# fkluger/vanishing_points_2017

Hardware: AMD Instinct MI355X
Metric: images/sec (LSD->CNN->EM) + horizon-AUC parity, YUD-shape, 1/2/4/8 GPU (higher is better)
Workload: dtype f32 (CNN: f32 operands / accumulation / results; conv1 multiply EXACT bf16 pieces of the f32 operands (three per operand) on the bf16 matrix cores; conv2-5, fc6 and fc7 multiply scaled fp16 PAIRS of the f32 operands (22 of 24 significand bits, three exact products per f32 product) on the fp16 matrix

## Files before the change

vanishing_points_2017_amd/csrc/em_device.hpp:

```cpp
#ifndef VPK_EM_DEVICE_HPP_
#define VPK_EM_DEVICE_HPP_

#include "wave_prims.hpp"
#include "../../include/vpk.h"
#include "em_layout.hpp"

namespace vpk {

constexpr int MAXM = 64;
constexpr int GRIDN = 20;
constexpr int NCELL = GRIDN * GRIDN;
constexpr int MAXCOMP = 100;
constexpr int MT = 8;
constexpr int PART_DOUBLES = 2048;
constexpr int WT_DOUBLES = 6144;
constexpr int KNN1 = 10;
constexpr int TRACE_COLS = 12;
constexpr int KNN2 = 4;
constexpr double PI_D = 3.141592653589793238462643383279502884;

struct Shared {
    double cur[MAXM * 3];
    double nxt[MAXM * 3];
    double s[MAXM];
    double pv[MAXM];
    double vx[MAXM], vy[MAXM];
    double k2[MAXM];
    double cnt[MAXM], cntw[MAXM], err[MAXM];
    int removed[MAXM];
    int icnt[MAXM];
    double red_v[32];
    int red_i[32];
    double pma[MAXCOMP], pmb[MAXCOMP], pw[MAXCOMP];
    float wts[NCELL];
    unsigned char mx[NCELL];
    int ncomp;
    int M;
    int status;
    unsigned flags;
    int ibuf[8];
    double dbuf[16];
    double sigma_prior;
    double active_us;
};

constexpr size_t SH_BYTES = (sizeof(Shared) + 15) / 16 * 16;
static_assert(sizeof(Shared) % 8 == 0 && sizeof(Shared) <= EM_STATE_DOUBLES * 8, "Shared must fit the slot's state region");
VPK_DEV Shared& SH() { return *reinterpret_cast<Shared*>(lds_base()); }
VPK_DEV double* WT() { return reinterpret_cast<double*>(lds_base() + SH_BYTES); }
VPK_DEV double* SCRATCH() { return WT(); }

struct EmCtx {
    int N;
    int ldn;
    int ld;
    int mcap;
    gdp l;
    cgdp lp;
    cgfp cnn;
    cgbp sphere;
    int ssize;
    cgdp init_vp;
    int n_init;
    vpk_em_params prm;
    gdp lsim;
    gdp pdist;
    gdp den;
    gdp lweight;
    gdp langle;
    gdp lscore;
    gdp lvsq;
    gdp pvl;
    gdp w;
    gdp wsrc;
    gdp drow;
    gdp cl;
    gip assoc;
    gip idx;
    gdp rowsum;
    int wt_doubles;
    gdp part;
    gdp lcopy;
    gdp lpcopy;
// ... 1233 lines not shown
        constexpr int RB = 4;
        const int nbatch = (M + RB - 1) / RB;
        for (int item = tid(); item < N * nbatch; item += nthreads()) {
            const int t0 = (item / N) * RB, kk = item - (item / N) * N;
            const double blw = bias * c.lweight[kk], dn = c.den[kk];
            cgdp pcol = c.part + kk;
            double v[RB][8];
#pragma unroll
            for (int u = 0; u < RB; ++u)
#pragma unroll
                for (int r = 0; r < 8; ++r)
                    v[u][r] = (t0 + u < M && r < R) ? pcol[((size_t)r * c.mcap + t0 + u) * c.ldn] : 0.0;
#pragma unroll
            for (int u = 0; u < RB; ++u) {
                if (t0 + u >= M) break;
                double sum = 0.0;
#pragma unroll
                for (int r = 0; r < 8; ++r) sum += v[u][r];
                c.w[(size_t)(m0 + t0 + u) * c.ldn + kk] = (wt[(size_t)kk * W + t0 + u] + blw * sum) / dn;
            }
        }
    }
    block_sync();
    if (tid() == 0) sh.dbuf[10] += lap(tq_);
}

VPK_DEVFN void zero_tail_rows(EmCtx& c) {
    const int N = c.N, jend = 8 * rs_jchunk(N);
    for (int p = tid(); p < (jend - N) * c.ld; p += nthreads()) c.lsim[(size_t)N * c.ld + p] = 0.0;
    block_sync();
}

template <int NT>
VPK_DEVFN void smooth_rows(EmCtx& c, int m0) {
    Shared& sh = SH();
    constexpr int W = NT * MT;
    constexpr int UNR = 4;
    const int N = uniform_int(c.N);
    m0 = uniform_int(m0);
    const int M = uniform_int(sh.M) - m0 < W ? uniform_int(sh.M) - m0 : W;
    const double bias = c.prm.wbias;
    double* wt = WT();
    long long tq_ = clock_ticks();
    const int jch = rs_jchunk(N), S = rs_sstride(jch, W);
    if (m0 != 0 || sh.ibuf[5] != RS_PANEL_FLAG + W) {
        for (int p = tid(); p < N * W; p += nthreads()) {
            const int j = p / W, m = p - j * W;
            wt[rs_row(j, jch, S, W) + m] = (m < M) ? c.wsrc[(size_t)j * c.mcap + m0 + m] : 0.0;
        }
        for (int p = N * W + tid(); p < 8 * jch * W; p += nthreads()) {
            const int j = p / W;
            wt[rs_row(j, jch, S, W) + (p - j * W)] = 0.0;
        }
        block_sync();
    }
    if (tid() == 0) sh.dbuf[8] += lap(tq_);
    double* red = wt + rs_panel_doubles(jch, W) + wave_id() * RS_RED_DOUBLES;
    const int d = lane() >> 4, i = lane() & 15;
    const int jA0 = d * jch, jB0 = (d + 4) * jch;
    const double* oA = wt + (size_t)d * S + i;
    const double* oB = wt + (size_t)(d + 4) * S + i;
    const size_t ld = (size_t)uniform_int(c.ld), ldn = (size_t)uniform_int(c.ldn);
    cgdp lsim = c.lsim, lweight = c.lweight, den = c.den;
    gdp wout = c.w;
    const int nb = (jch + UNR - 1) / UNR;
    cgdp lbase = uniform_ptr(lsim);
    const unsigned rowbytes = (unsigned)ld * 8u;
    const int kstep = uniform_int(nwaves()) * 16;
    int k0 = uniform_int(wave_id()) * 16;
    if (k0 < N) {
        int k = k0 + i;
        int kc = k < N ? k : N - 1;
        unsigned offA = ((unsigned)jA0 * (unsigned)ld + (unsigned)kc) * 8u, offB = ((unsigned)jB0 * (unsigned)ld + (unsigned)kc) * 8u;
        double aA[UNR], aB[UNR], nA_[UNR], nB_[UNR];
#pragma unroll
        for (int u = 0; u < UNR; ++u) {
            const int rn = u < jch ? u : jch - 1;
            cgdp rowp = (cgdp)((const VPK_GLOBAL char*)lbase + (size_t)rn * rowbytes);
            aA[u] = load_at(rowp, offA);
            aB[u] = load_at(rowp, offB);
        }
        for (;;) {
            const double lwk = lweight[kc];
            double dn = den[kc];
            const int k0n = k0 + kstep;
            const bool has_next = k0n < N;
            const int kn = k0n + i;
            const int kcn = has_next ? (kn < N ? kn : N - 1) : kc;
            const unsigned offAn = ((unsigned)jA0 * (unsigned)ld + (unsigned)kcn) * 8u, offBn = ((unsigned)jB0 * (unsigned)ld + (unsigned)kcn) * 8u;
            double accA[W], accB[W];
#pragma unroll
            for (int t = 0; t < W; ++t) { accA[t] = 0.0; accB[t] = 0.0; }
            double cA0 = oA[0], cA1 = W >= 24 ? oA[16] : 0.0, cB0 = oB[0], cB1 = W >= 24 ? oB[16] : 0.0;
            auto batch = [&](int b, double (&cuA)[UNR], double (&cuB)[UNR], double (&nxA)[UNR], double (&nxB)[UNR])
                             __attribute__((always_inline)) {
                const int r = b * UNR;
                const bool lastb = b + 1 == nb;
                const int nrow = lastb ? jch - r : UNR;
                const int rnext = lastb ? 0 : r + UNR;
                const unsigned oa = lastb ? offAn : offA, ob = lastb ? offBn : offB;
#pragma unroll
                for (int u = 0; u < UNR; ++u) {
                    int rn = rnext + u;
                    rn = rn < jch ? rn : jch - 1;
                    cgdp rowp = (cgdp)((const VPK_GLOBAL char*)lbase + (size_t)rn * rowbytes);
                    nxA[u] = load_at(rowp, oa);
                    nxB[u] = load_at(rowp, ob);
                }
#pragma unroll
                for (int u = 0; u < UNR; ++u) {
                    if (u < nrow) {
                        int rq = r + u + 1;
                        rq = rq < jch ? rq : 0;
                        const double* qA = oA + (size_t)rq * W;
                        const double* qB = oB + (size_t)rq * W;
                        const double xA0 = qA[0], xA1 = W >= 24 ? qA[16] : 0.0, xB0 = qB[0], xB1 = W >= 24 ? qB[16] : 0.0;
                        fmac8_row_bcast<0>(accA, cA0, cuA[u]);
                        if (W >= 16) fmac8_row_bcast<8>(accA + (W >= 16 ? 8 : 0), cA0, cuA[u]);
                        if (W >= 24) fmac8_row_bcast<0>(accA + (W >= 24 ? 16 : 0), cA1, cuA[u]);
// ... 196 lines not shown
            for (;;) {
                if (!step(va, vb)) break;
                if (!step(vb, va)) break;
            }
        }
    }
    if (tid() == 0) sh.dbuf[9] += lap(tq_);
#pragma unroll
    for (int cc = 0; cc < C; ++cc) {
        const int k = cc * WAVE + ln;
        if (k < N) {
#pragma unroll
            for (int q = 0; q < VPW; ++q) {
                const int t = wv + 8 * q;
                if (t < M) wout[(size_t)(m0 + t) * ldn + k] = (wreg[q][cc] + blwk[cc] * (tot[q][cc] + part[q][cc])) / dnk[cc];
            }
        }
    }
    block_sync();
    if (tid() == 0) sh.dbuf[10] += lap(tq_);
}
VPK_DEVFN void smooth_sparse_any(EmCtx& c, int m0) {
    switch (sp_cgroups(c.N)) {
        case 1: smooth_sparse<1>(c, m0); break;
        case 2: smooth_sparse<2>(c, m0); break;
        case 3: smooth_sparse<3>(c, m0); break;
        case 4: smooth_sparse<4>(c, m0); break;
        case 5: smooth_sparse<5>(c, m0); break;
        case 6: smooth_sparse<6>(c, m0); break;
        default: smooth_sparse<7>(c, m0); break;
    }
}

VPK_DEV void smooth_dispatch(EmCtx& c);
VPK_DEV void smooth(EmCtx& c) {
    smooth_dispatch(c);
    if (tid() == 0) SH().ibuf[5] = 0;
    block_sync();
}
VPK_DEV void smooth_dispatch(EmCtx& c) {
    Shared& sh = SH();
    const int M = sh.M, N = c.N;
    if (!c.prm.use_weights) {
        for (int m = 0; m < M; ++m)
            for (int k = tid(); k < N; k += nthreads()) c.w[(size_t)m * c.ldn + k] = c.wsrc[(size_t)k * c.mcap + m];
        block_sync();
        return;
    }
    if (M == 0) return;
    const int plan = smooth_plan(c, M);
    if (WAVE == 64 && (sh.ibuf[5] >= RS_PANEL_FLAG || plan == 2 || plan == 3)) {
        if (sparse_smoother_fits(c) && sh.ibuf[2] == 0) {
            for (int m0 = 0; m0 < M; m0 += 32) smooth_sparse_any(c, m0);
            return;
        }
        const int wpass = plan == 3 ? rs_wfit(c) : 32;
        for (int m0 = 0; m0 < M; m0 += wpass) {
            const int mm = (M - m0) < wpass ? (M - m0) : wpass;
            if (mm <= 8) smooth_rows<1>(c, m0);
            else if (mm <= 16) smooth_rows<2>(c, m0);
            else if (mm <= 24) smooth_rows<3>(c, m0);
            else smooth_rows<4>(c, m0);
        }
        return;
    }
    int wfit = (int)((c.wt_doubles / N) / MT) * MT;
    if (wfit > 32) wfit = 32;
    if (wfit >= MT) {
        for (int m0 = 0; m0 < M; m0 += wfit) {
            const int mm = (M - m0) < wfit ? (M - m0) : wfit;
            if (N > WAVE) {
                if (mm <= 8) smooth_full<1, 2>(c, m0);
                else if (mm <= 16) smooth_full<2, 2>(c, m0);
                else if (mm <= 24) smooth_full<3, 2>(c, m0);
                else smooth_full<4, 2>(c, m0);
            } else {
                if (mm <= 8) smooth_full<1, 1>(c, m0);
                else if (mm <= 16) smooth_full<2, 1>(c, m0);
                else if (mm <= 24) smooth_full<3, 1>(c, m0);
                else smooth_full<4, 1>(c, m0);
            }
        }
        return;
    }
    if (N > WAVE) smooth_blocks<2, 8>(c);
    else smooth_blocks<1, 4>(c);
}

VPK_DEVFN void assign_lines(EmCtx& c, bool hard) {
    Shared& sh = SH();
    const int M = sh.M, N = c.N;
    for (int n = tid(); n < N; n += nthreads()) {
        int best = 0;
        double bv = c.w[n];
        for (int m = 1; m < M; ++m) {
            double v = c.w[(size_t)m * c.ldn + n];
// ... 545 lines not shown
            } else {
                sh.flags |= VPK_EM_FLAG_VP_OVERFLOW;
            }
        }
    }
    if (tid() == 0) sh.dbuf[13] += lap(tq_);
    block_sync();
}

struct EmOut {
    double* vp;
    double* sigma;
    double* counts;
    double* counts_w;
    int* num_vp;
    long long* assoc;
    int* iterations;
    int* status;
    unsigned* flags;
    double* metric;
    double* trace;
    int max_vp;
    double* dbg = nullptr;
    double* d_pv = nullptr;
    double* d_angles = nullptr;
    double* d_pl = nullptr;
    double* d_plv = nullptr;
    double* d_pvl = nullptr;
    double* d_lvsq = nullptr;
};

VPK_DEVFN void write_result(EmCtx& c, EmOut& o, int status, int iterations) {
    Shared& sh = SH();
    const int N = c.N;
    int M = status == VPK_EM_OK ? sh.M : 0;
    if (M > o.max_vp) {
        M = o.max_vp;
        if (tid() == 0) sh.flags |= VPK_EM_FLAG_VP_OVERFLOW;
    }
    for (int m = tid(); m < o.max_vp; m += nthreads()) {
        bool ok = m < M;
        for (int d = 0; d < 3; ++d) o.vp[3 * m + d] = ok ? sh.nxt[3 * m + d] : 0.0;
        o.sigma[m] = ok ? sh.s[m] : 0.0;
        o.counts[m] = ok ? sh.cnt[m] : 0.0;
        o.counts_w[m] = ok ? sh.cntw[m] : 0.0;
    }
    for (int n = tid(); n < N; n += nthreads()) {
        int a = status == VPK_EM_OK ? c.assoc[n] : -1;
        o.assoc[n] = (a >= M) ? -1 : a;
        if (o.metric)
            for (int m = 0; m < o.max_vp; ++m)
                o.metric[(size_t)n * o.max_vp + m] = m < M ? c.w[(size_t)m * c.ldn + n] : 0.0;
    }
    if (o.d_pv) {
        for (int m = tid(); m < o.max_vp; m += nthreads()) {
            const bool ok = m < M;
            double alpha = 0.0, beta = 0.0;
            if (ok) {
                const double x0 = sh.nxt[3 * m], x1 = sh.nxt[3 * m + 1];
                beta = asin(x1);
                double inner = x0 / cos(beta);
                inner = inner < 1 ? inner : (is_nan(inner) ? inner : 1.0);
                inner = inner > -1 ? inner : (is_nan(inner) ? inner : -1.0);
                alpha = asin(inner);
            }
            o.d_pv[m] = ok ? sh.pv[m] : 0.0;
// ... 13 lines not shown
            }
            o.d_pl[n] = (pl > 1e-12 || is_nan(pl)) ? pl : 1e-12;
        }
    }
    block_sync();
    if (tid() == 0) {
        *o.num_vp = M;
        *o.iterations = iterations;
        *o.status = status;
        *o.flags = sh.flags;
    }
    block_sync();
}

VPK_DEV void trace_put(EmOut& o, int i, int slot, double v) {
    if (o.trace && tid() == 0) o.trace[TRACE_COLS * i + slot] = v;
}
VPK_DEV void trace_add(EmOut& o, int i, int slot, double v) {
    if (o.trace && tid() == 0) o.trace[TRACE_COLS * i + slot] += v;
}


constexpr int EM_DONE = 0, EM_SUSPENDED = 1;
constexpr long long EM_NO_DEADLINE = 0x7fffffffffffffffll;
struct EmSlice {
    long long deadline;
    int start_iter;
};

VPK_DEVFN void save_state(EmCtx& c) {
    typedef VPK_GLOBAL unsigned long long* gup;
    gup dst = (gup)c.state;
    const unsigned long long* src = reinterpret_cast<const unsigned long long*>(&SH());
    for (int q = tid(); q < (int)(sizeof(Shared) / 8); q += nthreads()) dst[q] = src[q];
    block_sync();
}
VPK_DEVFN void restore_state(EmCtx& c) {
    typedef const VPK_GLOBAL unsigned long long* cgup;
    cgup src = (cgup)c.state;
    unsigned long long* dst = reinterpret_cast<unsigned long long*>(&SH());
    block_sync();
    for (int q = tid(); q < (int)(sizeof(Shared) / 8); q += nthreads()) dst[q] = src[q];
    block_sync();
}

VPK_DEVFN int em_run(EmCtx& c, EmOut& o, EmSlice& sl) {
    Shared& sh = SH();
    const vpk_em_params& P = c.prm;
    const double max_stdd = 1e-6;
    const double merge_thresh_final = P.merge_thresh * 10;
    const int split_merge_it = 100;
    long long tk = clock_ticks();
    const long long t_begin = tk;
    int first = 0;
    if (sl.start_iter >= 0) {
        restore_state(c);
        first = sl.start_iter;
    } else {
    if (tid() == 0) { sh.flags = 0; sh.M = 0; sh.ncomp = 0; sh.ibuf[5] = 0; sh.ibuf[2] = 0; sh.active_us = 0; for (int q = 8; q < 16; ++q) sh.dbuf[q] = 0; }
    block_sync();
    if (o.trace)
        for (int q = tid(); q < TRACE_COLS * (P.num_iter + 1); q += nthreads()) o.trace[q] = 0.0;
    if (c.N <= 0) { write_result(c, o, VPK_EM_NO_VP, 0); return EM_DONE; }

    if (P.use_weights) { pairwise_setup(c, true); zero_tail_rows(c); }
    else pairwise_setup(c, false);
    trace_put(o, P.num_iter, 0, lap(tk));
    normalise_lines(c);
    for (int q = tid(); q < 3 * c.N; q += nthreads()) c.lcopy[q] = c.l[q];
    for (int q = tid(); q < 4 * c.N; q += nthreads()) c.lpcopy[q] = c.lp[q];
    block_sync();
    c.l = c.lcopy;
    c.lp = c.lpcopy;
    initial_vps(c);
    const int m_found = sh.M;
// ... 160 lines not shown
```

vanishing_points_2017_amd/csrc/vpk_core.hip:

```cpp
#include "vpk_internal.hpp"

#include <stdlib.h>
#include <string.h>

int vpk_fail(vpk_handle* h, int code, const char* what) {
    if (h) h->err = what;
    return code;
}
int vpk_fail_hip(vpk_handle* h, hipError_t e, const char* what) {
    if (h) h->err = std::string(what) + ": " + hipGetErrorString(e);
    return VPK_ERR_HIP;
}
int vpk_reserve(vpk_handle* h, void** p, size_t* have, size_t want, const char* what) {
    if (*have >= want && *p) return VPK_OK;
    if (*p) {
        VPK_HIP(h, hipStreamSynchronize(h->stream));
        VPK_HIP(h, hipFree(*p));
        *p = nullptr;
        *have = 0;
    }
    size_t grow = want + want / 8;
    hipError_t e = hipMalloc(p, grow);
    if (e != hipSuccess) {
        (void)hipGetLastError();
// ... 7 lines not shown

extern "C" {

int vpk_version(void) { return VPK_VERSION; }

int vpk_create(int device, vpk_handle** out) {
    if (!out) return VPK_ERR_ARG;
    *out = nullptr;
    int count = 0;
    if (hipGetDeviceCount(&count) != hipSuccess || count <= 0) return VPK_ERR_NO_DEVICE;
    if (device < 0 || device >= count) return VPK_ERR_ARG;
    hipDeviceProp_t prop;
    if (hipGetDeviceProperties(&prop, device) != hipSuccess) return VPK_ERR_HIP;
    if (strncmp(prop.gcnArchName, "gfx950", 6) != 0) {
        fprintf(stderr, "libvpk: device %d is %s; this library ships gfx950 (MI355X) code objects only\n",
                device, prop.gcnArchName);
        return VPK_ERR_NO_DEVICE;
    }
    if (hipSetDevice(device) != hipSuccess) return VPK_ERR_HIP;
    vpk_handle* h = new vpk_handle();
    h->device = device;
    h->num_cu = prop.multiProcessorCount;
    h->cu_share = h->num_cu;
    h->lds_per_block = (int)prop.sharedMemPerBlock;
    h->arch = 950;
    h->total_mem = prop.totalGlobalMem;
    if (hipStreamCreateWithFlags(&h->stream, hipStreamNonBlocking) != hipSuccess) {
        delete h;
        return VPK_ERR_HIP;
    }
    h->own_stream = true;
    if (const char* e = getenv("VPK_EM_WAIT_CAP")) { const int v = atoi(e); if (v >= 1 && v <= h->em_wait_cap) h->em_wait_cap = v; }
    if (const char* e = getenv("VPK_EM_STARTED_CAP")) { const int v = atoi(e); if (v >= 1 && v <= h->em_started_cap) h->em_started_cap = v; }
    *out = h;
    return VPK_OK;
}

int vpk_destroy(vpk_handle* h) {
    if (!h) return VPK_ERR_ARG;
    (void)hipSetDevice(h->device);
    (void)hipStreamSynchronize(h->stream);
    vpk_cnn_free(h);
    if (h->em_ws) (void)hipFree(h->em_ws);
    if (h->em_hdr) (void)hipFree(h->em_hdr);
    if (h->em_sess) (void)hipFree(h->em_sess);
    if (h->step_event) (void)hipEventDestroy(h->step_event);
    for (int i = 0; i < vpk_handle::VPK_HDR_RING; ++i) {
        if (h->em_hdr_host[i]) (void)hipHostFree(h->em_hdr_host[i]);
        if (h->em_hdr_ev[i]) (void)hipEventDestroy(h->em_hdr_ev[i]);
    }
    if (h->small_ws) (void)hipFree(h->small_ws);
    if (h->raster_hdr) (void)hipFree(h->raster_hdr);
    if (h->own_stream && h->stream) (void)hipStreamDestroy(h->stream);
    delete h;
    return VPK_OK;
}

int vpk_set_stream(vpk_handle* h, void* hip_stream) {
    if (!h) return VPK_ERR_ARG;
    VPK_HIP(h, hipStreamSynchronize(h->stream));
    if (h->own_stream && h->stream) {
        VPK_HIP(h, hipStreamDestroy(h->stream));
        h->own_stream = false;
        h->stream = nullptr;
    }
    if (hip_stream == nullptr) {
// ... 46 lines not shown
```

vanishing_points_2017_amd/csrc/vpk_em.hip:

```cpp
#include "em_device.hpp"
#include "vpk_internal.hpp"

#include <algorithm>
#include <string.h>
#include <numeric>
#include <vector>

using namespace vpk;

namespace {

constexpr int EM_THREADS = 512;
constexpr int EM_BOUND = EM_THREADS;
constexpr int EM_WAVES = EM_THREADS / 64;
constexpr size_t EM_LDS_BYTES = SH_BYTES + WT_DOUBLES * sizeof(double);
constexpr int WT_DOUBLES_BIG = (int)((163840 - SH_BYTES) / sizeof(double)) / 32 * 32;
constexpr size_t EM_LDS_BYTES_BIG = SH_BYTES + WT_DOUBLES_BIG * sizeof(double);
static_assert(EM_LDS_BYTES_BIG <= 163840, "LDS per CU");
#define VPK_SHARED_DECL Shared& sh = SH()

struct EmBatchArgs {
    int B;
    const long long* offsets;
    const int* order;
// ... 51 lines not shown
        int got = -1;
        const int start = (block_id() * 2) % ss.nslots;
        for (int sweep = 0; sweep < EM_SLOT_SWEEPS && got < 0; ++sweep) {
            for (int k = 0; k < ss.nslots && got < 0; ++k) {
                const int s = (start + k) % ss.nslots;
                if (atomicCAS(&ss.busy[s], 0, 1) == 0) got = s;
            }
            if (got < 0) __builtin_amdgcn_s_sleep(127);
        }
        sh.ibuf[7] = got;
    }
    block_sync();
    const int slot = sh.ibuf[7];
    block_sync();
    return slot;
}

VPK_DEV int pop_entry(int* head, const int* count) {
    Shared& sh = SH();
    if (tid() == 0) {
        int e = -1;
        const int n = *count;
        if (n > 0) { e = atomicAdd(head, 1); if (e >= n) e = -1; }
        sh.ibuf[7] = e;
    }
    block_sync();
    const int e = sh.ibuf[7];
    block_sync();
    return e;
}

__global__ __launch_bounds__(EM_BOUND) void em_batch_kernel(EmBatchArgs a, EmSliceArgs ss) {
    VPK_SHARED_DECL;
    const long long t_start = clock_ticks();
    const long long deadline = (ss.enabled && ss.budget_ticks > 0) ? t_start + ss.budget_ticks : EM_NO_DEADLINE;
    bool started_left = ss.enabled != 0, waiting_left = ss.enabled != 0;
    for (;;) {
        EmCtx c;
        EmOut o;
        EmSlice sl;
        sl.deadline = deadline;
        sl.start_iter = -1;
        int slot = -1;
        bool have = false;
        if (started_left) {
            const int e = pop_entry(&ss.ctr[0], &ss.ctr[1]);
            if (e >= 0) {
                const EmCarry& k = ss.in_started[e];
                c = k.c; o = k.o; sl.start_iter = k.iter; slot = k.slot;
                have = true;
            } else {
                started_left = false;
            }
        }
        if (!have && waiting_left) {
            const int e = pop_entry(&ss.ctr[3], &ss.ctr[4]);
            if (e >= 0) {
                const EmCarry& k = ss.in_waiting[e];
                c = k.c; o = k.o;
                have = true;
            } else {
                waiting_left = false;
            }
        }
        if (!have) {
            if (tid() == 0) sh.ibuf[7] = atomicAdd(a.queue, 1);
// ... 66 lines not shown
                if (tid() == 0) { *o.status = VPK_EM_NO_SLOT; *o.num_vp = 0; *o.iterations = 0; *o.flags = 0; }
                block_sync();
                continue;
            }
            bind_scratch(c, a.scratch + (size_t)slot * a.L.total_doubles, a.L, c.prm.do_split != 0);
        }
        int result = em_run(c, o, sl);
        while (result == EM_SUSPENDED) {
            if (tid() == 0) {
                int e = atomicAdd(&ss.ctr[2], 1);
                if (e < ss.cap_started) {
                    EmCarry& k = ss.out_started[e];
                    k.c = c; k.o = o; k.iter = sl.start_iter; k.slot = slot;
                } else {
                    e = -1;
                }
                sh.ibuf[7] = e;
            }
            block_sync();
            const bool parked = sh.ibuf[7] >= 0;
            block_sync();
            if (parked) break;
            sl.deadline = EM_NO_DEADLINE;
            result = em_run(c, o, sl);
        }
        if (result == EM_SUSPENDED) {
        } else if (ss.enabled) {
            block_sync();
            if (tid() == 0) { __threadfence(); atomicExch(&ss.busy[slot], 0); }
        }
    }
}

__global__ void em_rotate_kernel(int* ctr, int cap_waiting, int cap_started) {
    ctr[1] = ctr[2] < cap_started ? ctr[2] : cap_started;
    ctr[0] = 0;
    ctr[2] = 0;
    ctr[4] = ctr[5] < cap_waiting ? ctr[5] : cap_waiting;
    ctr[3] = 0;
    ctr[5] = 0;
}

__global__ __launch_bounds__(EM_BOUND) void pairwise_kernel(int n, const double* lp, EmLayout L, double* ws,
                                                              double* lsim_out, double* lscore_out,
                                                              double* langle_out, int smoother) {
    EmCtx c;
    c.N = n; c.lp = (cgdp)lp; c.wt_doubles = WT_DOUBLES; c.smoother = smoother;
    c.prm.use_weights = 1;
    bind_scratch(c, ws, L, false);
    pairwise_setup(c, true);
    for (int p = tid(); p < n * n; p += nthreads()) lsim_out[p] = c.lsim[(size_t)(p / n) * c.ld + p % n];
    for (int i = tid(); i < n; i += nthreads()) { lscore_out[i] = c.lscore[i]; langle_out[i] = c.langle[i]; }
}

__global__ __launch_bounds__(EM_BOUND) void init_vps_kernel(const float* cnn, const unsigned char* sphere,
                                                              int ssize, int num_max, double* v0_out,
                                                              int* m0_out, float* weights_out) {
    VPK_SHARED_DECL;
    EmCtx c;
    c.N = 0; c.cnn = (cgfp)cnn; c.sphere = (cgbp)sphere; c.ssize = ssize; c.wt_doubles = WT_DOUBLES;
    c.prm.num_init_vp = num_max;
    initial_vps(c);
    for (int k = tid(); k < 3 * sh.M; k += nthreads()) v0_out[k] = sh.cur[k];
    if (tid() == 0) *m0_out = sh.M;
    block_sync();
    prior_setup(c);
    for (int k = tid(); k < NCELL; k += nthreads()) weights_out[k] = sh.wts[k];
}

__global__ __launch_bounds__(EM_BOUND) void estep_kernel(int n, int m, const double* lp, const float* cnn,
                                                           const double* v, double* s, EmLayout L, double* ws,
                                                           double* p_v_out, double* lvsq_out, double* p_vl_out,
                                                           double* p_l_out) {
    VPK_SHARED_DECL;
    EmCtx c;
    c.N = n; c.lp = (cgdp)lp; c.cnn = (cgfp)cnn; c.wt_doubles = WT_DOUBLES;
    c.prm.use_weights = 1;
    bind_scratch(c, ws, L, false);
    prior_setup(c);
    for (int k = tid(); k < n; k += nthreads()) c.lweight[k] = 1.0;
    for (int k = tid(); k < 3 * m; k += nthreads()) sh.cur[k] = v[k];
    for (int k = tid(); k < m; k += nthreads()) sh.s[k] = s[k];
    if (tid() == 0) sh.M = m;
    block_sync();
    line_geometry_setup(c);
    estep(c, sh.cur);
    for (int k = tid(); k < m; k += nthreads()) { s[k] = sh.s[k]; p_v_out[k] = sh.pv[k]; }
    for (int p = tid(); p < m * n; p += nthreads()) {
        int k = p / n, q = p % n;
        lvsq_out[p] = c.lvsq[(size_t)k * c.ldn + q];
        p_vl_out[p] = c.pvl[(size_t)k * c.ldn + q];
    }
    for (int q = tid(); q < n; q += nthreads()) {
        double pl = 0.0;
        for (int k = 0; k < m; ++k) {
            double lv = c.lvsq[(size_t)k * c.ldn + q];
            pl += exp(-(lv / (2 * sh.s[k]))) * sh.k2[k] * sh.pv[k];
        }
        p_l_out[q] = (pl > 1e-12 || pl != pl) ? pl : 1e-12;
    }
}

__global__ __launch_bounds__(EM_BOUND) void weight_matrix_kernel(int n, int m, const double* p_vl,
                                                                   const double* lweight, const double* lsim,
                                                                   double bias, EmLayout L, double* ws,
                                                                   double* w_out, int smoother, int wt_doubles) {
    VPK_SHARED_DECL;
    EmCtx c;
    c.N = n; c.wt_doubles = wt_doubles; c.smoother = smoother;
    c.prm.use_weights = 1;
    c.prm.wbias = bias;
    bind_scratch(c, ws, L, false);
    for (int p = tid(); p < n * n; p += nthreads())
        c.lsim[(size_t)(p / n) * c.ld + p % n] = lsim[p];
    if (tid() == 0) { sh.M = m; sh.ibuf[5] = 0; sh.ibuf[2] = 0; }
    for (int i = tid(); i < n; i += nthreads()) c.lweight[i] = lweight[i];
    for (int p = tid(); p < m * n; p += nthreads()) c.pvl[(size_t)(p / n) * c.ldn + p % n] = p_vl[p];
    for (int p = tid(); p < n * c.mcap; p += nthreads()) {
        int i = p / c.mcap, k = p % c.mcap;
        c.wsrc[(size_t)i * c.mcap + k] = k < m ? p_vl[(size_t)k * n + i] * lweight[i] : 0.0;
    }
    block_sync();
    for (int k = tid(); k < n; k += nthreads()) {
        double sum = 0.0;
        for (int j = 0; j < n; ++j) sum += lsim[(size_t)j * n + k];
        c.den[k] = 1 + bias * c.lweight[k] * sum;
        if (!(fabs(sum) <= 1.7976931348623157e308)) sh.ibuf[2] = 1;
    }
    block_sync();
    zero_tail_rows(c);
    smooth(c);
    for (int p = tid(); p < m * n; p += nthreads()) w_out[p] = c.w[(size_t)(p / n) * c.ldn + p % n];
}

__global__ __launch_bounds__(EM_BOUND) void mstep_kernel(int n, int m, const double* l, const double* w,
                                                           EmLayout L, double* ws, double* vp_out,
                                                           int* valid_out) {
    VPK_SHARED_DECL;
    EmCtx c;
    c.N = n; c.l = (gdp) const_cast<double*>(l); c.wt_doubles = WT_DOUBLES;
    c.prm.s_thresh = 1e-200;
    bind_scratch(c, ws, L, false);
    if (tid() == 0) sh.M = m;
    for (int p = tid(); p < m * n; p += nthreads()) {
        int k = p / n, q = p % n;
        c.w[(size_t)k * c.ldn + q] = w[p];
        c.lvsq[(size_t)k * c.ldn + q] = 1.0;
        c.pvl[(size_t)k * c.ldn + q] = 1.0;
    }
    for (int k = tid(); k < 3 * m; k += nthreads()) { sh.cur[k] = (k % 3 == 2) ? 1.0 : 0.0; sh.nxt[k] = 0.0; }
    block_sync();
    mstep(c, 0, 1e-6);
    for (int k = tid(); k < m; k += nthreads()) {
        bool none = sh.removed[k] && sh.err[k] == -1.0 && !(sh.s[k] != sh.s[k]);
        valid_out[k] = none ? 0 : 1;
        for (int d = 0; d < 3; ++d) vp_out[3 * k + d] = none ? 0.0 : sh.nxt[3 * k + d];
    }
}

__global__ __launch_bounds__(EM_BOUND) void line_counts_kernel(int n, int m, const double* lp, const double* v,
                                                                 const double* s, const double* w, const double* lweight,
                                                                 double thresh, EmLayout L, double* ws, double* counts_out,
                                                                 double* counts_w_out, long long* assoc_out) {
    VPK_SHARED_DECL;
    EmCtx c;
    c.N = n; c.lp = (cgdp)lp; c.wt_doubles = WT_DOUBLES;
    c.prm.use_weights = 1;
    c.prm.outlier_thresh = thresh;
    bind_scratch(c, ws, L, false);
    for (int k = tid(); k < n; k += nthreads()) c.lweight[k] = lweight[k];
    for (int k = tid(); k < 3 * m; k += nthreads()) sh.cur[k] = v[k];
    for (int k = tid(); k < m; k += nthreads()) sh.s[k] = s[k];
    if (tid() == 0) { sh.M = m; sh.ncomp = 0; sh.sigma_prior = 1.0; }
    block_sync();
    line_geometry_setup(c);
    estep(c, sh.cur);
    for (int p = tid(); p < m * n; p += nthreads()) c.w[(size_t)(p / n) * c.ldn + p % n] = w[p];
    block_sync();
    assign_lines(c, true);
    count_lines(c);
    for (int k = tid(); k < m; k += nthreads()) { counts_out[k] = sh.cnt[k]; counts_w_out[k] = sh.cntw[k]; }
    for (int k = tid(); k < n; k += nthreads()) assoc_out[k] = c.assoc[k];
}

__global__ __launch_bounds__(EM_BOUND) void cluster2_kernel(int n, double* D, int* member, int* csize,
                                                              int* labels_out, unsigned* flags_out) {
    VPK_SHARED_DECL;
    if (tid() == 0) sh.flags = 0;
    block_sync();
    const int ld = n | 1;
    if (n <= CLUSTER_LDS_MAX && cluster_lds_doubles(n) <= WT_DOUBLES) {
        double* DL = WT();
        for (int p = tid(); p < n * n; p += nthreads()) {
            const int a = p / n, b = p % n;
            const double v = D[p];
            DL[a * ld + b] = (a == b || !(v + D[(size_t)b * n + a] != 0.0)) ? -1.0 : v;
        }
        block_sync();
        cluster2_lds(n);
        const int* lmember = cluster_lds_labels(DL, n);
        for (int q = tid(); q < n; q += nthreads()) member[q] = lmember[q];
        block_sync();
    } else {
        cluster2(sh, n, (gdp)D, (gip)member, (gip)csize);
    }
    for (int q = tid(); q < n; q += nthreads()) labels_out[q] = member[q];
    if (tid() == 0) *flags_out = sh.flags;
}

template <typename K>
int allow_lds(vpk_handle* h, K kernel) {
    VPK_HIP(h, hipFuncSetAttribute(reinterpret_cast<const void*>(kernel),
                                   hipFuncAttributeMaxDynamicSharedMemorySize, (int)EM_LDS_BYTES_BIG));
    return VPK_OK;
}
int em_prepare(vpk_handle* h) {
    if (h->em_ready) return VPK_OK;
    int rc;
    if ((rc = allow_lds(h, em_batch_kernel))) return rc;
    if ((rc = allow_lds(h, pairwise_kernel))) return rc;
    if ((rc = allow_lds(h, init_vps_kernel))) return rc;
    if ((rc = allow_lds(h, estep_kernel))) return rc;
    if ((rc = allow_lds(h, weight_matrix_kernel))) return rc;
    if ((rc = allow_lds(h, mstep_kernel))) return rc;
    if ((rc = allow_lds(h, cluster2_kernel))) return rc;
    if ((rc = allow_lds(h, line_counts_kernel))) return rc;
    h->em_ready = true;
    return VPK_OK;
}

struct EmMode { int per_cu; int wt_doubles; size_t lds_bytes; };
EmMode em_mode(const vpk_handle* h) {
    if (h->em_lds_doubles <= 0) return EmMode{1, WT_DOUBLES_BIG, EM_LDS_BYTES_BIG};
    const int wt = std::min(std::max(h->em_lds_doubles, 64), WT_DOUBLES_BIG);
    return EmMode{1, wt, SH_BYTES + (size_t)std::max(wt, PART_DOUBLES) * sizeof(double)};
}

int em_slots(const vpk_handle* h, int batch, size_t slot_bytes, int per_cu) {
    int slots = h->cu_share * per_cu;
    if (h->em_max_workgroups > 0 && slots > h->em_max_workgroups) slots = h->em_max_workgroups;
    if (slots > batch) slots = batch;
    size_t budget = h->total_mem / 2;
    while (slots > 1 && (size_t)slots * slot_bytes > budget) slots /= 2;
    return slots < 1 ? 1 : slots;
}

int check_params(vpk_handle* h, const vpk_em_params* p, int n_init, bool has_init) {
    if (!p) return vpk_fail(h, VPK_ERR_ARG, "params is null");
    if (p->num_iter < 1 || p->num_iter > 100000) return vpk_fail(h, VPK_ERR_ARG, "num_iter out of range");
    if (p->split_merge_freq < 1) return vpk_fail(h, VPK_ERR_ARG, "split_merge_freq < 1");
    if (p->num_init_vp < 1 || p->num_init_vp > MAXM) return vpk_fail(h, VPK_ERR_LIMIT, "num_init_vp must be 1..64");
    if (has_init && (n_init < 1 || n_init > MAXM)) return vpk_fail(h, VPK_ERR_LIMIT, "n_init must be 1..64");
    return VPK_OK;
}

constexpr size_t EM_SESS_HEAD = 256;

struct SessView { int* ctr; int* busy; EmCarry* started[2]; EmCarry* waiting[2]; };
SessView sess_view(vpk_handle* h) {
    char* base = (char*)h->em_sess;
    SessView v;
    v.ctr = (int*)base;
    v.busy = (int*)(base + EM_SESS_HEAD);
    char* p = base + EM_SESS_HEAD + em_align((size_t)h->em_sess_slots * 4, 256);
    const size_t sb = em_align(sizeof(EmCarry) * h->em_started_cap, 256), wb = em_align(sizeof(EmCarry) * h->em_wait_cap, 256);
    v.started[0] = (EmCarry*)p; v.started[1] = (EmCarry*)(p + sb);
    v.waiting[0] = (EmCarry*)(p + 2 * sb); v.waiting[1] = (EmCarry*)(p + 2 * sb + wb);
    return v;
}
size_t sess_bytes(const vpk_handle* h, int slots) {
    return EM_SESS_HEAD + em_align((size_t)slots * 4, 256) + 2 * em_align(sizeof(EmCarry) * h->em_started_cap, 256) +
           2 * em_align(sizeof(EmCarry) * h->em_wait_cap, 256);
}
EmSliceArgs sess_next(vpk_handle* h, double slice_ms) {
    SessView v = sess_view(h);
    hipLaunchKernelGGL(em_rotate_kernel, dim3(1), dim3(1), 0, h->stream, v.ctr, h->em_wait_cap, h->em_started_cap);
    h->em_sess_in ^= 1;
    EmSliceArgs ss;
    ss.enabled = 1;
    ss.budget_ticks = slice_ms > 0 ? (long long)(slice_ms * 1e-3 / (CLOCK_US * 1e-6)) : 0;
    if (slice_ms > 0 && ss.budget_ticks < 1) ss.budget_ticks = 1;
    ss.ctr = v.ctr;
    ss.in_started = v.started[h->em_sess_in]; ss.out_started = v.started[h->em_sess_in ^ 1];
    ss.in_waiting = v.waiting[h->em_sess_in]; ss.out_waiting = v.waiting[h->em_sess_in ^ 1];
    ss.cap_started = h->em_started_cap; ss.cap_waiting = h->em_wait_cap;
    ss.busy = v.busy; ss.nslots = h->em_sess_slots;
    return ss;
}

int em_flush(vpk_handle* h) {
    if (!h->em_unflushed) return VPK_OK;
    EmSliceArgs ss = sess_next(h, 0.0);
    EmBatchArgs a = {};
    a.B = 0;
    a.queue = ss.ctr + 8;
    a.L = h->em_sess_layout;
    a.scratch = (double*)h->em_ws;
    a.wt_doubles = h->em_sess_wt_doubles;
    a.smoother = h->em_smoother;
    hipLaunchKernelGGL(em_batch_kernel, dim3(h->em_sess_wgs), dim3(EM_THREADS), h->em_sess_lds, h->stream, a, ss);
    VPK_HIP(h, hipGetLastError());
    h->em_unflushed = false;
    return VPK_OK;
}

EmLayout small_layout(int n, int m) {
    return em_layout(n, (int)em_align((size_t)(m > 0 ? m : 1), 8), EM_WAVES, true, false);
}

}

namespace {
__global__ void math_probe_kernel(int fn, long long n, const double* __restrict__ x, double* __restrict__ y) {
    const long long i = (long long)blockIdx.x * blockDim.x + threadIdx.x;
    if (i >= n) return;
    const double v = x[i];
    double r;
    switch (fn) {
        case 0: r = exp(v); break;
        case 1: r = acos(v); break;
        case 2: r = asin(v); break;
        case 3: r = atan(v); break;
        case 4: r = sqrt(v); break;
        case 5: r = sin(v); break;
        case 6: r = cos(v); break;
        default: r = log(v); break;
    }
    y[i] = r;
}
}

extern "C" {

int vpk_math_probe(vpk_handle* h, int fn, long long n, const double* x, double* y) {
// ... 283 lines not shown
```

vanishing_points_2017_amd/csrc/vpk_internal.hpp:

```cpp
#ifndef VPK_INTERNAL_HPP_
#define VPK_INTERNAL_HPP_

#include <vector>
#include <hip/hip_runtime.h>
#include <stdio.h>
#include <string>

#include "../../include/vpk.h"
#include "em_layout.hpp"

struct vpk_cnn_state;

struct vpk_handle {
    int device = 0;
    hipStream_t stream = nullptr;
    bool own_stream = false;
    std::string err;
    int num_cu = 0;
    int cu_share = 0;
    int em_max_workgroups = 0;
    int em_smoother = 0;
    int em_lds_doubles = 0;
    int em_wait_cap = 8192;
    int em_started_cap = 1024;
    int lds_per_block = 0;
    int arch = 0;
    size_t total_mem = 0;
    void* em_ws = nullptr;
    size_t em_ws_bytes = 0;
    void* em_hdr = nullptr;
    size_t em_hdr_bytes = 0;
    static constexpr int VPK_HDR_RING = 4;
    void* em_hdr_host[VPK_HDR_RING] = {};
    size_t em_hdr_host_bytes[VPK_HDR_RING] = {};
    hipEvent_t em_hdr_ev[VPK_HDR_RING] = {};
    bool em_hdr_ev_valid[VPK_HDR_RING] = {};
    int em_hdr_next = 0;
    void* small_ws = nullptr;
    size_t small_ws_bytes = 0;
    bool raster_ready = false;
    void* raster_hdr = nullptr;
    size_t raster_hdr_bytes = 0;
    std::vector<long long> raster_offsets;
    int raster_table_size = 0;
    int raster_last_batch = 0;
    int raster_alternative = 0;
    bool em_ready = false;
    double em_slice_ms = 0.0;
    vpk_em_dist_out em_dist = {};
    bool em_dist_set = false;
    int em_slice_nmax = 0;
    void* em_sess = nullptr;
    size_t em_sess_bytes = 0;
    int em_sess_in = 0;
    bool em_unflushed = false;
    size_t em_sess_slot_bytes = 0;
    int em_sess_slots = 0;
// ... 21 lines not shown
```

Baseline: 22280.

## Split straggler EM smoothing across teams of workgroups during session flush

Adds a team kernel that runs at flush time after a short time-sliced first pass. Leftover started EM problems are handed to teams of up to eight workgroups. Each team member copies the slot scratch, smooths a disjoint range of line columns, and the members sync through a global-memory barrier with double-buffered weight outputs. The aim is to stop a few long EM tails from leaving most CUs idle at the end of a batch. The cost is extra scratch copies, global barriers with timeouts, slot pressure, and added complexity.

```diff
diff --git a/vanishing_points_2017_amd/csrc/em_device.hpp b/vanishing_points_2017_amd/csrc/em_device.hpp
--- a/vanishing_points_2017_amd/csrc/em_device.hpp
+++ b/vanishing_points_2017_amd/csrc/em_device.hpp
@@ -42,6 +42,16 @@
     double dbuf[16];
     double sigma_prior;
     double active_us;
+    struct Team {
+        int on;
+        int T, r;
+        int gen;
+        int failed;
+        unsigned* bar;
+        double* wx[2];
+        double* wown;
+        int pad_;
+    } tm;
 };
 
 constexpr size_t SH_BYTES = (sizeof(Shared) + 15) / 16 * 16;
@@ -49,6 +59,14 @@
 VPK_DEV Shared& SH() { return *reinterpret_cast<Shared*>(lds_base()); }
 VPK_DEV double* WT() { return reinterpret_cast<double*>(lds_base() + SH_BYTES); }
 VPK_DEV double* SCRATCH() { return WT(); }
+constexpr size_t SH_STATE_WORDS = offsetof(Shared, tm) / 8;
+static_assert(offsetof(Shared, tm) % 8 == 0, "Shared::tm is 8-byte aligned");
+constexpr int EM_TEAM_ON = 0x7ea70001;
+VPK_DEV bool team_on(const Shared& sh) { return sh.tm.on == EM_TEAM_ON && sh.tm.T > 1; }
+VPK_DEV void team_solo() {
+    if (tid() == 0) { Shared::Team& t = SH().tm; t.on = 0; t.T = 1; t.r = 0; t.gen = 0; t.failed = 0; t.bar = nullptr; t.wx[0] = t.wx[1] = nullptr; t.wown = nullptr; }
+    block_sync();
+}
 
 struct EmCtx {
     int N;
@@ -1348,7 +1366,7 @@
 }
 
 template <int NT>
-VPK_DEVFN void smooth_rows(EmCtx& c, int m0) {
+VPK_DEVFN void smooth_rows(EmCtx& c, int m0, int kb, int ke) {
     Shared& sh = SH();
     constexpr int W = NT * MT;
     constexpr int UNR = 4;
@@ -1383,8 +1401,9 @@
     cgdp lbase = uniform_ptr(lsim);
     const unsigned rowbytes = (unsigned)ld * 8u;
     const int kstep = uniform_int(nwaves()) * 16;
-    int k0 = uniform_int(wave_id()) * 16;
-    if (k0 < N) {
+    ke = uniform_int(ke);
+    int k0 = uniform_int(kb) + uniform_int(wave_id()) * 16;
+    if (k0 < ke) {
         int k = k0 + i;
         int kc = k < N ? k : N - 1;
         unsigned offA = ((unsigned)jA0 * (unsigned)ld + (unsigned)kc) * 8u, offB = ((unsigned)jB0 * (unsigned)ld + (unsigned)kc) * 8u;
@@ -1400,7 +1419,7 @@
             const double lwk = lweight[kc];
             double dn = den[kc];
             const int k0n = k0 + kstep;
-            const bool has_next = k0n < N;
+            const bool has_next = k0n < ke;
             const int kn = k0n + i;
             const int kcn = has_next ? (kn < N ? kn : N - 1) : kc;
             const unsigned offAn = ((unsigned)jA0 * (unsigned)ld + (unsigned)kcn) * 8u, offBn = ((unsigned)jB0 * (unsigned)ld + (unsigned)kcn) * 8u;
@@ -1663,6 +1682,40 @@
     }
 }
 
+constexpr long long EM_TEAM_WAIT_TICKS = (long long)(1.0e6 / CLOCK_US);
+VPK_DEVFN void team_barrier() {
+#if defined(__HIPCC__)
+    Shared& sh = SH();
+    asm volatile("s_waitcnt vmcnt(0)" ::: "memory");
+    block_sync();
+    if (tid() == 0) {
+        Shared::Team& t = sh.tm;
+        const unsigned target = (unsigned)(++t.gen) * (unsigned)t.T;
+        __builtin_amdgcn_fence(__ATOMIC_RELEASE, "agent");
+        asm volatile("s_waitcnt vmcnt(0)" ::: "memory");
+        __hip_atomic_fetch_add(t.bar, 1u, __ATOMIC_RELAXED, __HIP_MEMORY_SCOPE_AGENT);
+        if (!t.failed) {
+            const long long dl = clock_ticks() + EM_TEAM_WAIT_TICKS;
+            while (__hip_atomic_load(t.bar, __ATOMIC_RELAXED, __HIP_MEMORY_SCOPE_AGENT) < target) {
+                if (clock_ticks() > dl) { t.failed = 1; __hip_atomic_store(t.bar + 1, 1u, __ATOMIC_RELAXED, __HIP_MEMORY_SCOPE_AGENT); break; }
+                __builtin_amdgcn_s_sleep(2);
+            }
+        }
+        __builtin_amdgcn_fence(__ATOMIC_ACQUIRE, "agent");
+        asm volatile("s_waitcnt vmcnt(0)" ::: "memory");
+    }
+    block_sync();
+#endif
+}
+VPK_DEV void team_columns(EmCtx& c, int& kb, int& ke) {
+    const Shared::Team& t = SH().tm;
+    const int nb = (c.N + 15) >> 4;
+    const int b0 = (int)((long long)nb * t.r / t.T), b1 = (int)((long long)nb * (t.r + 1) / t.T);
+    kb = 16 * b0;
+    ke = 16 * b1 < c.N ? 16 * b1 : c.N;
+    c.w = (gdp)t.wx[(t.gen + 1) & 1];
+}
+
 VPK_DEV void smooth_dispatch(EmCtx& c);
 VPK_DEV void smooth(EmCtx& c) {
     smooth_dispatch(c);
@@ -1672,6 +1725,7 @@
 VPK_DEV void smooth_dispatch(EmCtx& c) {
     Shared& sh = SH();
     const int M = sh.M, N = c.N;
+    if (team_on(sh)) c.w = (gdp)sh.tm.wown;
     if (!c.prm.use_weights) {
         for (int m = 0; m < M; ++m)
             for (int k = tid(); k < N; k += nthreads()) c.w[(size_t)m * c.ldn + k] = c.wsrc[(size_t)k * c.mcap + m];
@@ -1685,14 +1739,18 @@
             for (int m0 = 0; m0 < M; m0 += 32) smooth_sparse_any(c, m0);
             return;
         }
+        int kb = 0, ke = N;
+        const bool team = team_on(sh);
+        if (team) team_columns(c, kb, ke);
         const int wpass = plan == 3 ? rs_wfit(c) : 32;
         for (int m0 = 0; m0 < M; m0 += wpass) {
             const int mm = (M - m0) < wpass ? (M - m0) : wpass;
-            if (mm <= 8) smooth_rows<1>(c, m0);
-            else if (mm <= 16) smooth_rows<2>(c, m0);
-            else if (mm <= 24) smooth_rows<3>(c, m0);
-            else smooth_rows<4>(c, m0);
-        }
+            if (mm <= 8) smooth_rows<1>(c, m0, kb, ke);
+            else if (mm <= 16) smooth_rows<2>(c, m0, kb, ke);
+            else if (mm <= 24) smooth_rows<3>(c, m0, kb, ke);
+            else smooth_rows<4>(c, m0, kb, ke);
+        }
+        if (team) team_barrier();
         return;
     }
     int wfit = (int)((c.wt_doubles / N) / MT) * MT;
@@ -2304,6 +2362,7 @@
 
 VPK_DEVFN void write_result(EmCtx& c, EmOut& o, int status, int iterations) {
     Shared& sh = SH();
+    if (team_on(sh) && sh.tm.r != 0) return;
     const int N = c.N;
     int M = status == VPK_EM_OK ? sh.M : 0;
     if (M > o.max_vp) {
@@ -2383,7 +2442,7 @@
     typedef VPK_GLOBAL unsigned long long* gup;
     gup dst = (gup)c.state;
     const unsigned long long* src = reinterpret_cast<const unsigned long long*>(&SH());
-    for (int q = tid(); q < (int)(sizeof(Shared) / 8); q += nthreads()) dst[q] = src[q];
+    for (int q = tid(); q < (int)SH_STATE_WORDS; q += nthreads()) dst[q] = src[q];
     block_sync();
 }
 VPK_DEVFN void restore_state(EmCtx& c) {
@@ -2391,7 +2450,7 @@
     cgup src = (cgup)c.state;
     unsigned long long* dst = reinterpret_cast<unsigned long long*>(&SH());
     block_sync();
-    for (int q = tid(); q < (int)(sizeof(Shared) / 8); q += nthreads()) dst[q] = src[q];
+    for (int q = tid(); q < (int)SH_STATE_WORDS; q += nthreads()) dst[q] = src[q];
     block_sync();
 }
 
diff --git a/vanishing_points_2017_amd/csrc/vpk_core.hip b/vanishing_points_2017_amd/csrc/vpk_core.hip
--- a/vanishing_points_2017_amd/csrc/vpk_core.hip
+++ b/vanishing_points_2017_amd/csrc/vpk_core.hip
@@ -63,6 +63,7 @@
     h->own_stream = true;
     if (const char* e = getenv("VPK_EM_WAIT_CAP")) { const int v = atoi(e); if (v >= 1 && v <= h->em_wait_cap) h->em_wait_cap = v; }
     if (const char* e = getenv("VPK_EM_STARTED_CAP")) { const int v = atoi(e); if (v >= 1 && v <= h->em_started_cap) h->em_started_cap = v; }
+    if (const char* e = getenv("VPK_EM_FLUSH_TEAM")) { const int v = atoi(e); if (v >= 1 && v <= 64) h->em_flush_team = v; }
     *out = h;
     return VPK_OK;
 }
diff --git a/vanishing_points_2017_amd/csrc/vpk_em.hip b/vanishing_points_2017_amd/csrc/vpk_em.hip
--- a/vanishing_points_2017_amd/csrc/vpk_em.hip
+++ b/vanishing_points_2017_amd/csrc/vpk_em.hip
@@ -107,6 +107,7 @@
 
 __global__ __launch_bounds__(EM_BOUND) void em_batch_kernel(EmBatchArgs a, EmSliceArgs ss) {
     VPK_SHARED_DECL;
+    team_solo();
     const long long t_start = clock_ticks();
     const long long deadline = (ss.enabled && ss.budget_ticks > 0) ? t_start + ss.budget_ticks : EM_NO_DEADLINE;
     bool started_left = ss.enabled != 0, waiting_left = ss.enabled != 0;
@@ -239,6 +240,144 @@
     }
 }
 
+struct EmTeamRec {
+    unsigned join;
+    unsigned size;
+    unsigned bar[2];
+    int xslot;
+    unsigned pad[11];
+};
+static_assert(sizeof(EmTeamRec) == 64, "one record per 64 bytes");
+constexpr unsigned EM_TEAM_CLOSED = 0x80000000u;
+constexpr long long EM_TEAM_FORM_TICKS = (long long)(20.0 / CLOCK_US);
+struct EmTeamArgs {
+    EmTeamRec* rec;
+    unsigned* head;
+    int cap;
+};
+
+VPK_DEV void release_slot(const EmSliceArgs& ss, int slot) {
+    block_sync();
+    if (tid() == 0) { __threadfence(); atomicExch(&ss.busy[slot], 0); }
+}
+
+__global__ __launch_bounds__(EM_BOUND) void em_team_kernel(EmBatchArgs a, EmSliceArgs ss, EmTeamArgs ta) {
+    VPK_SHARED_DECL;
+    team_solo();
+    const int P = ss.ctr[1];
+    const int G = (int)gridDim.x;
+    int T = P > 0 ? G / P : 1;
+    T = T < 1 ? 1 : (T > ta.cap ? ta.cap : T);
+    const size_t slot_doubles = a.L.total_doubles;
+    int spare = -1;
+    {
+        const int b = block_id();
+        int e = (b / (8 * T)) * 8 + b % 8;
+        bool own = true;
+        for (;;) {
+            if (!own || e >= P) {
+                own = false;
+                if (tid() == 0) sh.ibuf[7] = (int)atomicAdd(ta.head, 1u);
+                block_sync();
+                e = sh.ibuf[7];
+                block_sync();
+                if (e >= P) break;
+            }
+            own = false;
+            if (spare < 0) { spare = acquire_slot(ss); if (spare < 0) break; }
+            EmTeamRec* R = ta.rec + e;
+            if (tid() == 0) {
+                const unsigned old = atomicAdd(&R->join, 1u);
+                int pos = (old & EM_TEAM_CLOSED) ? -1 : (int)old;
+                unsigned n = 0;
+                int xs = spare;
+                if (pos == 0) {
+                    const long long dl = clock_ticks() + EM_TEAM_FORM_TICKS;
+                    while ((__hip_atomic_load(&R->join, __ATOMIC_RELAXED, __HIP_MEMORY_SCOPE_AGENT) & ~EM_TEAM_CLOSED) < (unsigned)T &&
+                           clock_ticks() < dl)
+                        __builtin_amdgcn_s_sleep(2);
+                    n = atomicOr(&R->join, EM_TEAM_CLOSED) & ~EM_TEAM_CLOSED;
+                    if (n > (unsigned)ta.cap) n = (unsigned)ta.cap;
+                    R->xslot = spare;
+                    __builtin_amdgcn_fence(__ATOMIC_RELEASE, "agent");
+                    asm volatile("s_waitcnt vmcnt(0)" ::: "memory");
+                    __hip_atomic_store(&R->size, n, __ATOMIC_RELAXED, __HIP_MEMORY_SCOPE_AGENT);
+                } else if (pos > 0) {
+                    const long long dl = clock_ticks() + EM_TEAM_WAIT_TICKS;
+                    while ((n = __hip_atomic_load(&R->size, __ATOMIC_RELAXED, __HIP_MEMORY_SCOPE_AGENT)) == 0 && clock_ticks() < dl)
+                        __builtin_amdgcn_s_sleep(2);
+                    __builtin_amdgcn_fence(__ATOMIC_ACQUIRE, "agent");
+                    asm volatile("s_waitcnt vmcnt(0)" ::: "memory");
+                    if (n == 0 || (unsigned)pos >= n) pos = -1;
+                    else xs = R->xslot;
+                }
+                sh.ibuf[4] = pos; sh.ibuf[5] = (int)n; sh.ibuf[6] = xs;
+            }
+            block_sync();
+            const int pos = sh.ibuf[4], n = sh.ibuf[5], xs = sh.ibuf[6];
+            block_sync();
+            if (pos < 0) continue;
+            const EmCarry& k = ss.in_started[e];
+            EmCtx c = k.c;
+            EmOut o = k.o;
+            EmSlice sl;
+            sl.deadline = EM_NO_DEADLINE;
+            sl.start_iter = k.iter;
+            if (pos > 0) {
+                gdp own_base = (gdp)(a.scratch + (size_t)spare * slot_doubles);
+                cgdp src = (cgdp)(a.scratch + (size_t)k.slot * slot_doubles);
+                for (size_t q = tid(); q < slot_doubles; q += nthreads()) own_base[q] = src[q];
+                bind_scratch(c, a.scratch + (size_t)spare * slot_doubles, a.L, c.prm.do_split != 0);
+                c.l = c.lcopy;
+                c.lp = c.lpcopy;
+                o.trace = nullptr;
+                o.dbg = nullptr;
+            }
+            if (tid() == 0) {
+                Shared::Team& t = sh.tm;
+                double* xb = a.scratch + (size_t)xs * slot_doubles;
+                t.on = EM_TEAM_ON; t.T = n; t.r = pos; t.gen = 0; t.failed = 0;
+                t.bar = R->bar;
+                t.wx[0] = xb + a.L.w; t.wx[1] = xb + a.L.pvl;
+                t.wown = (double*)(void*)c.w;
+            }
+            team_barrier();
+            em_run(c, o, sl);
+            team_barrier();
+            if (pos == 0) {
+                const bool failed = sh.tm.failed || __hip_atomic_load(R->bar + 1, __ATOMIC_RELAXED, __HIP_MEMORY_SCOPE_AGENT) != 0;
+                if (failed && tid() == 0) { *o.status = VPK_EM_NO_SLOT; *o.num_vp = 0; *o.iterations = 0; *o.flags = 0; }
+                release_slot(ss, k.slot);
+                release_slot(ss, spare);
+            } else {
+                release_slot(ss, spare);
+            }
+            spare = -1;
+            team_solo();
+        }
+    }
+    if (spare >= 0) release_slot(ss, spare);
+    for (;;) {
+        const int e = pop_entry(&ss.ctr[3], &ss.ctr[4]);
+        if (e < 0) break;
+        const EmCarry& k = ss.in_waiting[e];
+        EmCtx c = k.c;
+        EmOut o = k.o;
+        EmSlice sl;
+        sl.deadline = EM_NO_DEADLINE;
+        sl.start_iter = -1;
+        const int slot = acquire_slot(ss);
+        if (slot < 0) {
+            if (tid() == 0) { *o.status = VPK_EM_NO_SLOT; *o.num_vp = 0; *o.iterations = 0; *o.flags = 0; }
+            block_sync();
+            continue;
+        }
+        bind_scratch(c, a.scratch + (size_t)slot * slot_doubles, a.L, c.prm.do_split != 0);
+        em_run(c, o, sl);
+        release_slot(ss, slot);
+    }
+}
+
 __global__ void em_rotate_kernel(int* ctr, int cap_waiting, int cap_started) {
     ctr[1] = ctr[2] < cap_started ? ctr[2] : cap_started;
     ctr[0] = 0;
@@ -264,6 +403,7 @@
                                                               int ssize, int num_max, double* v0_out,
                                                               int* m0_out, float* weights_out) {
     VPK_SHARED_DECL;
+    team_solo();
     EmCtx c;
     c.N = 0; c.cnn = (cgfp)cnn; c.sphere = (cgbp)sphere; c.ssize = ssize; c.wt_doubles = WT_DOUBLES;
     c.prm.num_init_vp = num_max;
@@ -280,6 +420,7 @@
                                                            double* p_v_out, double* lvsq_out, double* p_vl_out,
                                                            double* p_l_out) {
     VPK_SHARED_DECL;
+    team_solo();
     EmCtx c;
     c.N = n; c.lp = (cgdp)lp; c.cnn = (cgfp)cnn; c.wt_doubles = WT_DOUBLES;
     c.prm.use_weights = 1;
@@ -313,6 +454,7 @@
                                                                    double bias, EmLayout L, double* ws,
                                                                    double* w_out, int smoother, int wt_doubles) {
     VPK_SHARED_DECL;
+    team_solo();
     EmCtx c;
     c.N = n; c.wt_doubles = wt_doubles; c.smoother = smoother;
     c.prm.use_weights = 1;
@@ -344,6 +486,7 @@
                                                            EmLayout L, double* ws, double* vp_out,
                                                            int* valid_out) {
     VPK_SHARED_DECL;
+    team_solo();
     EmCtx c;
     c.N = n; c.l = (gdp) const_cast<double*>(l); c.wt_doubles = WT_DOUBLES;
     c.prm.s_thresh = 1e-200;
@@ -370,6 +513,7 @@
                                                                  double thresh, EmLayout L, double* ws, double* counts_out,
                                                                  double* counts_w_out, long long* assoc_out) {
     VPK_SHARED_DECL;
+    team_solo();
     EmCtx c;
     c.N = n; c.lp = (cgdp)lp; c.wt_doubles = WT_DOUBLES;
     c.prm.use_weights = 1;
@@ -393,6 +537,7 @@
 __global__ __launch_bounds__(EM_BOUND) void cluster2_kernel(int n, double* D, int* member, int* csize,
                                                               int* labels_out, unsigned* flags_out) {
     VPK_SHARED_DECL;
+    team_solo();
     if (tid() == 0) sh.flags = 0;
     block_sync();
     const int ld = n | 1;
@@ -425,6 +570,7 @@
     if (h->em_ready) return VPK_OK;
     int rc;
     if ((rc = allow_lds(h, em_batch_kernel))) return rc;
+    if ((rc = allow_lds(h, em_team_kernel))) return rc;
     if ((rc = allow_lds(h, pairwise_kernel))) return rc;
     if ((rc = allow_lds(h, init_vps_kernel))) return rc;
     if ((rc = allow_lds(h, estep_kernel))) return rc;
@@ -463,7 +609,7 @@
 
 constexpr size_t EM_SESS_HEAD = 256;
 
-struct SessView { int* ctr; int* busy; EmCarry* started[2]; EmCarry* waiting[2]; };
+struct SessView { int* ctr; int* busy; EmCarry* started[2]; EmCarry* waiting[2]; char* team; size_t team_bytes; };
 SessView sess_view(vpk_handle* h) {
     char* base = (char*)h->em_sess;
     SessView v;
@@ -473,11 +619,13 @@
     const size_t sb = em_align(sizeof(EmCarry) * h->em_started_cap, 256), wb = em_align(sizeof(EmCarry) * h->em_wait_cap, 256);
     v.started[0] = (EmCarry*)p; v.started[1] = (EmCarry*)(p + sb);
     v.waiting[0] = (EmCarry*)(p + 2 * sb); v.waiting[1] = (EmCarry*)(p + 2 * sb + wb);
+    v.team = p + 2 * sb + 2 * wb;
+    v.team_bytes = 256 + sizeof(EmTeamRec) * (size_t)h->em_started_cap;
     return v;
 }
 size_t sess_bytes(const vpk_handle* h, int slots) {
     return EM_SESS_HEAD + em_align((size_t)slots * 4, 256) + 2 * em_align(sizeof(EmCarry) * h->em_started_cap, 256) +
-           2 * em_align(sizeof(EmCarry) * h->em_wait_cap, 256);
+           2 * em_align(sizeof(EmCarry) * h->em_wait_cap, 256) + 256 + sizeof(EmTeamRec) * (size_t)h->em_started_cap;
 }
 EmSliceArgs sess_next(vpk_handle* h, double slice_ms) {
     SessView v = sess_view(h);
@@ -495,9 +643,11 @@
     return ss;
 }
 
+constexpr double EM_FLUSH_FIRST_MS = 1.0;
 int em_flush(vpk_handle* h) {
     if (!h->em_unflushed) return VPK_OK;
-    EmSliceArgs ss = sess_next(h, 0.0);
+    const bool teams = h->em_flush_team > 1;
+    EmSliceArgs ss = sess_next(h, teams ? EM_FLUSH_FIRST_MS : 0.0);
     EmBatchArgs a = {};
     a.B = 0;
     a.queue = ss.ctr + 8;
@@ -507,6 +657,17 @@
     a.smoother = h->em_smoother;
     hipLaunchKernelGGL(em_batch_kernel, dim3(h->em_sess_wgs), dim3(EM_THREADS), h->em_sess_lds, h->stream, a, ss);
     VPK_HIP(h, hipGetLastError());
+    if (teams) {
+        ss = sess_next(h, 0.0);
+        const SessView v = sess_view(h);
+        VPK_HIP(h, hipMemsetAsync(v.team, 0, v.team_bytes, h->stream));
+        EmTeamArgs ta;
+        ta.head = (unsigned*)v.team;
+        ta.rec = (EmTeamRec*)(v.team + 256);
+        ta.cap = h->em_flush_team;
+        hipLaunchKernelGGL(em_team_kernel, dim3(h->em_sess_wgs), dim3(EM_THREADS), h->em_sess_lds, h->stream, a, ss, ta);
+        VPK_HIP(h, hipGetLastError());
+    }
     h->em_unflushed = false;
     return VPK_OK;
 }
diff --git a/vanishing_points_2017_amd/csrc/vpk_internal.hpp b/vanishing_points_2017_amd/csrc/vpk_internal.hpp
--- a/vanishing_points_2017_amd/csrc/vpk_internal.hpp
+++ b/vanishing_points_2017_amd/csrc/vpk_internal.hpp
@@ -23,6 +23,7 @@
     int em_lds_doubles = 0;
     int em_wait_cap = 8192;
     int em_started_cap = 1024;
+    int em_flush_team = 8;
     int lds_per_block = 0;
     int arch = 0;
     size_t total_mem = 0;
```

Measured after the change: 22590, median of 6. 1.01x the previous value.
